# adelacvg/NS2VC

Measured on NVIDIA H100. Metric: denoiser-steps/s, higher is better.
Workload: dtype f32 (3xBF16-split tensor-core contractions, fp32 accumulate)

## Files before the change

ns2vc_b200/csrc/common.cuh:

```cuda
#pragma once
#include <cuda_runtime.h>
#include <cuda_bf16.h>
#include <stdint.h>
#include <stddef.h>

namespace ns2vc {

void set_error(const char* fmt, ...);
const char* get_error();

#define NS_CHECK_CUDA(expr)                                                                    \
  do {                                                                                         \
    cudaError_t _e = (expr);                                                                   \
    if (_e != cudaSuccess) {                                                                   \
      ns2vc::set_error("%s:%d CUDA error %s: %s", __FILE__, __LINE__, cudaGetErrorName(_e),    \
                       cudaGetErrorString(_e));                                                \
      return -2;                                                                               \
    }                                                                                          \
  } while (0)

#define NS_REQUIRE(cond, ...)                                                                  \
  do {                                                                                         \
    if (!(cond)) {                                                                             \
      ns2vc::set_error(__VA_ARGS__);                                                           \
// ... 102 lines not shown
  double* row_stats;
  int f16_col0;
  double* stat_sum;
  double* stat_sq;
  unsigned long long* trace;
  unsigned long long* span;
  int tma_out;
  int bn;
  int xmode;
  int ksplit;
  int nxs;
  XSeg xs[kMaxXSeg];
  const PrepOp* pre;
  const float* pre_film;
  const float* rowmask;
  const int* row_len;
  int len_shift;
  TMap tmap[2 * kMaxSrc];
  TMap tmap_out[3];
};
void plan_gemm(GemmOp& op);
constexpr int kXfMaxC = 1024;
int gemm_sm_count();

int launch_gemm_tc(const GemmOp& op, cudaStream_t st);
int launch_gemm_simt(const GemmOp& op, cudaStream_t st);
int encode_tmaps(GemmOp& op);

struct PackSeg {
  const float* w;
  int n_rows;
  int cin_total;
  int ktaps;
  int tap;
  int cin0, ncin;
  int n_dst0;
  int kb0;
  int nkb;
  int geglu_half;
  const float* cscale;
};
int launch_pack_b(const PackSeg& ps, __nv_bfloat16* w_hi, __nv_bfloat16* w_lo, float* w_f32, int Npad,
                  cudaStream_t st);
int launch_ln_fold_vec(const float* W, const float* gamma, const float* beta, const float* bias, float* g, float* bf, int N, int C, cudaStream_t st);

int launch_prep_split(const PrepOp& op, cudaStream_t st);
// ... 128 lines not shown
```

ns2vc_b200/csrc/gemm_tc.cu:

```cuda
#include "gemm_common.cuh"
#include "prep_common.cuh"
#include "tc_common.cuh"
#include "launch.cuh"
#include <cuda.h>
#include <cuda_fp16.h>
#include <cstdlib>

namespace ns2vc {

constexpr int BM = 128;
constexpr int BK = 64;
constexpr int kEpiWarps = 8;
constexpr int kThreads = (4 + kEpiWarps) * 32;
constexpr int kATileBytes = BM * BK * 2;

constexpr int kMaxStages = 4;
constexpr int kStagePerWarp = 8192;
constexpr int kStageOff = 8192;
constexpr int kStagingBytes = kStageOff + kEpiWarps * kStagePerWarp;

constexpr int kPanelRows = BM + 2;
constexpr int kPanelBytes = 136 * 128;
constexpr int kXAStageBytes = 2 * kPanelBytes;
constexpr int kXBStageBytes = 3 * 2 * (64 * BK * 2);
constexpr int kXAStages = 3;
constexpr int kXBStages = 2;
constexpr int kXOffB = kXAStages * kXAStageBytes;
constexpr int kXOffAff = kXOffB + kXBStages * kXBStageBytes;
constexpr int kXAffBytes = (2 * kXfMaxC + 2 * 64) * 4;

template <int BN_> struct TileCfg {
  static constexpr int BN = BN_;
  static constexpr int kBTileBytes = BN_ * BK * 2;
  static constexpr int kStageBytes = 2 * kATileBytes + 2 * kBTileBytes;
  static constexpr int kStagesSingle = (BN_ == 128) ? 3 : 4;
  static constexpr int kOffAcc = kStagingBytes;
  static constexpr int kPipeBytes = (kStagesSingle * kStageBytes > kXOffAff + kXAffBytes) ? kStagesSingle * kStageBytes : kXOffAff + kXAffBytes;
  static constexpr int kOffBar = kPipeBytes;
  static constexpr int kOffDesc = kOffBar + 1024;
  static constexpr int kOffLnG = kOffDesc + 3072;
  static constexpr int kSmemBytes = kOffLnG + 4096 + 1024 ;
};
static_assert(TileCfg<64>::kSmemBytes <= 227 * 1024 && TileCfg<128>::kSmemBytes <= 227 * 1024, "shared memory budget");
static_assert(kXOffAff + kXAffBytes <= TileCfg<64>::kPipeBytes && kPrepSlots * kEpiWarps * 32 >= kXfMaxC, "panel mode: stages + affine table inside the pipeline area");
constexpr int kXOffAcc = kXOffB + 8 * 256 * 16;
static_assert(kXOffAcc + BM * 64 * 4 <= kXOffAff, "panel mode: parked accumulator inside the weight ring");
static_assert(TileCfg<64>::kOffAcc + BM * 64 * 4 <= TileCfg<64>::kStagesSingle * TileCfg<64>::kStageBytes &&
              TileCfg<128>::kOffAcc + BM * 128 * 4 <= TileCfg<128>::kStagesSingle * TileCfg<128>::kStageBytes, "parked accumulator inside the stage buffers");


__device__ __forceinline__ float* stage_f32_ptr(uint8_t* st, int row, int c4) {
  return reinterpret_cast<float*>(st + row * 128 + ((c4 ^ (row & 7)) << 4));
}


template <bool LNF, bool VOC = false>
__device__ __noinline__ void epi_cold(const GemmOp& op, int b, long long m, int nbase, uint8_t* st, int lane, bool with_gate) {
#pragma unroll 1
  for (int j = 0; j < 32; ++j) {
    float* pv = stage_f32_ptr(st, lane, j >> 2) + (j & 3);
    const float g = with_gate ? reinterpret_cast<const float*>(st + 4096)[lane * 32 + j] : 0.f;
    *pv = (nbase + j < op.n_valid) ? epi_value<LNF, VOC>(op, b, m, nbase + j, *pv, g) : 0.f;
  }
}
__device__ __noinline__ void store_cold(const GemmOp& op, int flags, int b, int t, long long m, int nbase, uint8_t* st, int lane) {
  const bool f16 = nbase >= op.f16_col0;
#pragma unroll 1
  for (int j = 0; j < 32; ++j) {
    const int n = nbase + j;
    if (n >= op.n_valid) break;
    const float v = stage_f32_ptr(st, lane, j >> 2)[j & 3];
// ... 50 lines not shown
      const uint32_t sa = smem_u32(st);
      if (tma & 1) tma_store_3d(&tmo[0], sa, nbase, t_warp0, b);
      if (tma & 2) { tma_store_3d(&tmo[1], sa + 4096u, nbase, t_warp0, b); tma_store_3d(&tmo[2], sa + 6144u, nbase, t_warp0, b); }
      bulk_commit();
    }
  }
  const int direct = ((op.flags & EPI_OUT_NCT) ? EPI_OUT_NCT : 0) | (((op.flags & EPI_OUT_F32) && !(op.tma_out & 1)) ? EPI_OUT_F32 : 0) |
                     (((op.flags & EPI_OUT_SPLIT) && with_split && !(op.tma_out & 2)) ? EPI_OUT_SPLIT : 0);
  if (direct) {
    if (!stage_f32) park_row(st, lane, val);
    if (mv) store_cold(op, direct, b, t, m, nbase, st, lane);
  }
}

__device__ __forceinline__ unsigned long long gtime() { unsigned long long t; asm volatile("mov.u64 %0, %%globaltimer;" : "=l"(t)); return t; }
#define XTRACE(i) do { if (op_param.trace && blockIdx.x == 0 && tid == 128) op_param.trace[16 + (i)] = gtime(); } while (0)
#define TRACE(i) do { if (op.trace && blockIdx.x == 0 && blockIdx.y == 0) op.trace[i] = gtime(); } while (0)
__device__ __forceinline__ long long gclk() { long long t; asm volatile("mov.u64 %0, %%clock64;" : "=l"(t)); return t; }
#define ETRACE(i) do { if (op.trace && blockIdx.x == 0 && blockIdx.y == 0 && warp == 4 && lane == 0) op.trace[8 + (i)] = gclk(); } while (0)

constexpr int kGemmOpHotBytes = (int)offsetof(GemmOp, tmap);
static_assert(kGemmOpHotBytes % 16 == 0 && kGemmOpHotBytes <= 2688 && sizeof(PrepOp) <= 320, "GemmOp's hot part must fit the shared-memory descriptor copy");

template <int BN_, bool LNF, bool XF, bool ENC = false, bool RAG = false, bool VOC = false>
__global__ void __launch_bounds__(kThreads, 1) gemm_tc_kernel(const __grid_constant__ GemmOp op_param) {
  using Cfg = TileCfg<BN_>;
  constexpr int BN = Cfg::BN;
  constexpr int kStageBytes = Cfg::kStageBytes;
  extern __shared__ uint8_t smem_raw[];
  const uint32_t raw = smem_u32(smem_raw);
  const uint32_t base = (raw + 1023u) & ~1023u;
  uint8_t* smem = smem_raw + (base - raw);
  const uint32_t bar_base = base + Cfg::kOffBar;
  auto full_bar = [&](int s) { return bar_base + 8u * s; };
  auto empty_bar = [&](int s) { return bar_base + 8u * (kMaxStages + s); };
  auto b_full = [&](int s) { return bar_base + 8u * (19 + s); };
  auto b_empty = [&](int s) { return bar_base + 8u * (21 + s); };

  const int tid = threadIdx.x, warp = tid >> 5, lane = tid & 31;
  {
    const uint4* src = reinterpret_cast<const uint4*>(&op_param);
    uint4* dst = reinterpret_cast<uint4*>(smem + Cfg::kOffDesc);
    for (int i = tid; i < kGemmOpHotBytes / 16; i += kThreads) dst[i] = src[i];
    if (XF && op_param.xmode && op_param.pre) {
      const uint4* ps = reinterpret_cast<const uint4*>(op_param.pre);
      uint4* pd = reinterpret_cast<uint4*>(smem + Cfg::kOffDesc + 2688);
      for (int i = tid; i < (int)(sizeof(PrepOp) / 16); i += kThreads) pd[i] = __ldg(ps + i);
    }
  }
  const GemmOp& op = *reinterpret_cast<const GemmOp*>(smem + Cfg::kOffDesc);
  const TMap* tmaps = op_param.tmap;
  const int tiles_per_batch = (op_param.T_out + BM - 1) / BM;
  const int n_tiles = op_param.N / BN;
  const int ks = (XF && op_param.xmode && op_param.ksplit > 1) ? op_param.ksplit : 1;
  const int kr = (int)blockIdx.x % ks, bid = (int)blockIdx.x / ks;
  const int nst = Cfg::kStagesSingle;
  uint8_t* stage_area = smem;
  float* acc_tile = reinterpret_cast<float*>(smem + (XF ? kXOffAcc : Cfg::kOffAcc));
  const int wg = (warp - 4) >> 2;
  float acc_d[BN / 2];
#pragma unroll
  for (int i = 0; i < BN / 2; ++i) acc_d[i] = 0.f;
  auto mma3 = [&](uint32_t a_hi, uint32_t a_lo, uint32_t b_hi, uint32_t b_lo) {
    wgmma_bf16<BN>(acc_d, wg_desc(a_hi), wg_desc(b_hi));
    wgmma_bf16<BN>(acc_d, wg_desc(a_lo), wg_desc(b_hi));
    wgmma_bf16<BN>(acc_d, wg_desc(a_hi), wg_desc(b_lo));
  };
  const int nkb = op_param.nkb_total;
  const bool tr0 = blockIdx.x == 0;
  auto xr_ready = [&]() { return bar_base + 8u * 23; };
  auto xr_full = [&]() { return bar_base + 8u * 24; };
  if (tid == 0 && op_param.trace && tr0) op_param.trace[0] = gtime();
  span_begin(op_param.span);

  if (warp == 1 && lane == 0) {
    for (int s = 0; s < kMaxStages; ++s) { mbar_init(full_bar(s), 1); mbar_init(empty_bar(s), kEpiWarps); }
    if (XF) { mbar_init(xr_ready(), 1); mbar_init(xr_full(), kEpiWarps); for (int a = 0; a < kXBStages; ++a) { mbar_init(b_full(a), 1); mbar_init(b_empty(a), kEpiWarps); } }
    mbar_fence_init();
  }
  if (warp == 0 && lane == 0) {
// ... 143 lines not shown
          wgmma_fence();
          for (int j = 0; j < xs.ntap; ++j) {
#pragma unroll
            for (int k = 0; k < BK / 16; ++k) {
              const uint32_t bh = b0 + j * 2 * Cfg::kBTileBytes + k * 32;
              mma3(a_hi + j * 128 + k * 32, a_lo + j * 128 + k * 32, bh, bh + Cfg::kBTileBytes);
            }
          }
          wgmma_commit();
          wgmma_wait<1>();
          if (it > 0 && lane == 0) { mbar_arrive(empty_bar((it - 1) % kXAStages)); mbar_arrive(b_empty((it - 1) % kXBStages)); }
          ++it;
        }
      }
      wgmma_wait<0>();
      XTRACE(4);
    }
  }

  const int npf = nkb < nst ? nkb : nst;
  if constexpr (!xpanel) if (warp == 0 && elect_one()) {
    const int n0 = (bid % n_tiles) * BN;
    for (int kb = 0; kb < npf; ++kb) {
      const uint32_t b_hi = base + kb * kStageBytes + 2 * kATileBytes;
      mbar_arrive_expect_tx(full_bar(kb), 2u * kATileBytes + 2u * Cfg::kBTileBytes);
      const size_t eoff = ((size_t)kb * op.N + n0) * 64;
      bulk_g2s(b_hi, op.w_hi + eoff, Cfg::kBTileBytes, full_bar(kb));
      bulk_g2s(b_hi + Cfg::kBTileBytes, op.w_lo + eoff, Cfg::kBTileBytes, full_bar(kb));
    }
  }
  __syncwarp();

  if (warp == 0) {
    if constexpr (!xpanel) if (elect_one()) {
      const int npre = npf;
      pdl_wait();
      if (tr0) TRACE(2);
      {
        const int mt = bid / n_tiles, n0 = (bid % n_tiles) * BN;
        const int b = mt / tiles_per_batch, t0 = (mt % tiles_per_batch) * BM;
        int si = 0, kbl = 0;
        for (int kb = 0; kb < nkb; ++kb) {
          const int stage = kb % nst;
          const GSeg& s = op.seg[si];
          const uint32_t a_hi = base + stage * kStageBytes;
          const uint32_t a_lo = a_hi + kATileBytes;
          const uint32_t b_hi = a_lo + kATileBytes;
          if (kb >= npre) {
            if (kb >= nst) mbar_wait(empty_bar(stage), (uint32_t)(((kb / nst) & 1) ^ 1));
            mbar_arrive_expect_tx(full_bar(stage), 2u * kATileBytes + 2u * Cfg::kBTileBytes);
            const size_t eoff = ((size_t)kb * op.N + n0) * 64;
            bulk_g2s(b_hi, op.w_hi + eoff, Cfg::kBTileBytes, full_bar(stage));
            bulk_g2s(b_hi + Cfg::kBTileBytes, op.w_lo + eoff, Cfg::kBTileBytes, full_bar(stage));
          }
          const int c = s.c0 + kbl * 64;
          tma_load_3d(a_hi, &tmaps[2 * s.src], c, t0 + s.tap, b, full_bar(stage));
          tma_load_3d(a_lo, &tmaps[2 * s.src + 1], c, t0 + s.tap, b, full_bar(stage));
          if (++kbl == s.nkb) { kbl = 0; ++si; }
        }
      }
    }
  } else if (warp >= 4) {
    pdl_wait();
    __syncwarp();
    const bool leader = elect_one();
    const int q = warp & 3;
    const int r = q * 32 + lane;
    const int cc0 = (warp - 4) >> 2;
    uint8_t* st = stage_area + kStageOff + (warp - 4) * kStagePerWarp;
    const TMap* tmo = op_param.tmap_out;
    bool staged_once = false;
    {
      constexpr int it = 0;
      const int mt = bid / n_tiles, nt = bid % n_tiles, n0 = nt * BN;
      const int b = mt / tiles_per_batch, t0 = (mt % tiles_per_batch) * BM;
      const int t = t0 + r;
      const bool mv = t < op.T_out;
      const long long m = (long long)b * op.T_out + t;
      bool rv = mv;
      if constexpr (RAG) rv = mv && t < ragged_rows(op.row_len, b, op.len_shift);
      if constexpr (VOC) if (op.flags & EPI_ROWMASK) rv = mv && __ldg(op.rowmask + m) != 0.f;
      if constexpr (!xpanel) {
        for (int kb = 0; kb < nkb; ++kb) {
          const int stage = kb % nst;
          mbar_wait(full_bar(stage), (uint32_t)((kb / nst) & 1));
          if (kb == 0 && tr0 && warp == 4 && lane == 0) TRACE(3);
          const uint32_t a_hi = base + stage * kStageBytes + wg * 64 * 128;
          const uint32_t a_lo = a_hi + kATileBytes;
          const uint32_t b_hi = base + stage * kStageBytes + 2 * kATileBytes;
          wgmma_fence();
#pragma unroll
          for (int k = 0; k < BK / 16; ++k) mma3(a_hi + k * 32, a_lo + k * 32, b_hi + k * 32, b_hi + Cfg::kBTileBytes + k * 32);
          wgmma_commit();
          wgmma_wait<1>();
          if (kb > 0 && lane == 0) mbar_arrive(empty_bar((kb - 1) % nst));
        }
        wgmma_wait<0>();
        if (lane == 0) mbar_arrive(empty_bar((nkb - 1) % nst));
        if (it == 0 && tr0 && warp == 4 && lane == 0) TRACE(4);
      }
      asm volatile("bar.sync 1, 256;" ::: "memory");
      acc_park<BN>(acc_tile, acc_d, wg, tid & 127);
#pragma unroll
      for (int i = 0; i < BN / 2; ++i) acc_d[i] = 0.f;
      asm volatile("bar.sync 1, 256;" ::: "memory");
      const int t_warp0 = t0 + q * 32;
      float pre[32];
      float preg[32];
      bool pre_ok = false;
      float ln_mu = 0.f, ln_rstd = 1.f;
      float* sg = reinterpret_cast<float*>(smem + Cfg::kOffLnG) + (warp - 4) * 128;
      if constexpr (LNF) {
        if (mv) ln_row_stats(op, m, ln_mu, ln_rstd);
        __syncwarp();
        if constexpr (BN == 128) {
          const int nb = nt * 64 + cc0 * 32 + lane;
          const bool ok = nb < op.n_valid;
          sg[lane] = ok ? __ldg(op.ln_g + nb) : 0.f;
          sg[32 + lane] = ok ? __ldg(op.ln_g + op.n_valid + nb) : 0.f;
          sg[64 + lane] = ok ? __ldg(op.bias + nb) : 0.f;
          sg[96 + lane] = ok ? __ldg(op.bias + op.n_valid + nb) : 0.f;
          pre_ok = BN == 128 && nt * 64 + cc0 * 32 + 32 <= op.n_valid;
        } else {
          const int nb = n0 + cc0 * 32 + lane;
          const bool ok = nb < op.n_valid;
          sg[lane] = ok ? __ldg(op.ln_g + nb) : 0.f;
          sg[64 + lane] = (ok && (op.flags & EPI_BIAS)) ? __ldg(op.bias + nb) : 0.f;
          pre_ok = mv && n0 + cc0 * 32 + 32 <= op.n_valid && !(op.flags & (EPI_ROWBIAS | EPI_RESIDUAL));
        }
        __syncwarp();
      }
      if constexpr (!LNF) {
      if constexpr (BN == 128) {
        const int nb = nt * 64 + cc0 * 32;
        if (BN == 128 && nb + 32 <= op.n_valid) {
          pre_ok = true;
          const float4* bv = reinterpret_cast<const float4*>(op.bias + nb);
          const float4* bg = reinterpret_cast<const float4*>(op.bias + op.n_valid + nb);
#pragma unroll
          for (int j = 0; j < 8; ++j) {
            const float4 x = __ldg(bv + j), y = __ldg(bg + j);
            pre[4 * j] = x.x; pre[4 * j + 1] = x.y; pre[4 * j + 2] = x.z; pre[4 * j + 3] = x.w;
            preg[4 * j] = y.x; preg[4 * j + 1] = y.y; preg[4 * j + 2] = y.z; preg[4 * j + 3] = y.w;
          }
        }
      } else {
        const int nb = n0 + cc0 * 32;
        if (mv && nb + 32 <= op.n_valid && !(op.flags & EPI_ROWBIAS) && (!(op.flags & EPI_RESIDUAL) || (op.res_ld & 3) == 0)) {
          pre_ok = true;
#pragma unroll
          for (int j = 0; j < 32; ++j) pre[j] = 0.f;
          if (op.flags & EPI_BIAS) {
            const float4* pb = reinterpret_cast<const float4*>(op.bias + nb);
#pragma unroll
            for (int j = 0; j < 8; ++j) { const float4 v = __ldg(pb + j); pre[4 * j] = v.x; pre[4 * j + 1] = v.y; pre[4 * j + 2] = v.z; pre[4 * j + 3] = v.w; }
          }
          if (op.flags & EPI_RESIDUAL) {
            const float4* pr = reinterpret_cast<const float4*>(op.res + m * op.res_ld + nb);
#pragma unroll
            for (int j = 0; j < 8; ++j) { const float4 v = __ldg(pr + j); pre[4 * j] += v.x; pre[4 * j + 1] += v.y; pre[4 * j + 2] += v.z; pre[4 * j + 3] += v.w; }
          }
        }
      }
      }
      float enc_keep = 1.f;
      if constexpr (ENC) if ((op.flags & EPI_ROWMASK) && mv) enc_keep = __ldg(op.rowmask + m);
      if (it == 0 && tr0 && warp == 4 && lane == 0) TRACE(5);
      if (it == 0 && tr0) ETRACE(0);
      auto wait_staging = [&]() {
        if (staged_once && op.tma_out) {
          if (leader) asm volatile("cp.async.bulk.wait_group.read 0;" ::: "memory");
          __syncwarp();
        }
      };
      if constexpr (BN == 128) {
        {
          const int hh = cc0;
          float val[32], gate[32];
          acc_row32<BN>(acc_tile, r, hh * 32, val);
          acc_row32<BN>(acc_tile, r, 64 + hh * 32, gate);
          const int nbase = nt * 64 + hh * 32;
          if (nbase < op.n_valid) {
            if (!rv) {
#pragma unroll
              for (int j = 0; j < 32; ++j) val[j] = 0.f;
            } else if (pre_ok) {
              if constexpr (LNF) {
#pragma unroll
                for (int j = 0; j < 32; j += 2) {
                  const float v0 = fmaf(ln_rstd, val[j] - ln_mu * sg[j], sg[64 + j]), v1 = fmaf(ln_rstd, val[j + 1] - ln_mu * sg[j + 1], sg[65 + j]);
                  const float g0 = fmaf(ln_rstd, gate[j] - ln_mu * sg[32 + j], sg[96 + j]), g1 = fmaf(ln_rstd, gate[j + 1] - ln_mu * sg[33 + j], sg[97 + j]);
                  upk2(fmul2(pk2(v0, v1), gelu_erf2(pk2(g0, g1))), val[j], val[j + 1]);
                }
              } else {
#pragma unroll
                for (int j = 0; j < 32; j += 2)
                  upk2(fmul2(fadd2(pk2(val[j], val[j + 1]), pk2(pre[j], pre[j + 1])), gelu_erf2(fadd2(pk2(gate[j], gate[j + 1]), pk2(preg[j], preg[j + 1])))),
                       val[j], val[j + 1]);
              }
            } else {
              wait_staging();
              park_row(st, lane, val);
#pragma unroll
              for (int j = 0; j < 8; ++j) reinterpret_cast<float4*>(st + 4096)[lane * 8 + j] = make_float4(gate[4 * j], gate[4 * j + 1], gate[4 * j + 2], gate[4 * j + 3]);
              epi_cold<LNF>(op, b, m, nbase, st, lane, true);
              fetch_row(st, lane, val);
            }
            wait_staging();
            emit_chunk(op, tmo, st, lane, leader, false, b, t, t_warp0, m, mv, nbase, val);
            staged_once = true;
          }
        }
      } else {
        float* sm_part = reinterpret_cast<float*>(stage_area) + (it & 1) * (4 * BN * 2);
        const bool stage_f32 = (op.tma_out & 1) || (op.flags & EPI_STATS);
#pragma unroll 1
        for (int cc = cc0; cc < BN / 32; cc += 2) {
          float acc[32];
          acc_row32<BN>(acc_tile, r, cc * 32, acc);
          if (it == 0 && tr0) ETRACE(1);
          if constexpr (XF) if (ks > 1) {
            const int te = tid - 128;
            if (kr != 0) {
              mbar_wait_cluster(xr_ready(), 0);
              const uint32_t rbase = mapa_u32(base + kXOffB, 0);
#pragma unroll
              for (int j = 0; j < 8; ++j) st_remote_f32x4(rbase + (uint32_t)((j * 256 + te) * 16), acc[4 * j], acc[4 * j + 1], acc[4 * j + 2], acc[4 * j + 3]);
              asm volatile("fence.acq_rel.cluster;" ::: "memory");
              __syncwarp();
              if (lane == 0) mbar_arrive_remote(mapa_u32(xr_full(), 0));
              continue;
            }
            if (warp == 4 && lane == 0) mbar_arrive_remote(mapa_u32(xr_ready(), 1));
            mbar_wait_cluster(xr_full(), 0);
            const float4* xr = reinterpret_cast<const float4*>(smem + kXOffB);
#pragma unroll
            for (int j = 0; j < 8; ++j) {
              const float4 v = xr[j * 256 + te];
              acc[4 * j] += v.x; acc[4 * j + 1] += v.y; acc[4 * j + 2] += v.z; acc[4 * j + 3] += v.w;
            }
          }
          const int nbase = n0 + cc * 32;
// ... 66 lines not shown
              for (int rr = 0; rr < 32; ++rr) { const float v = stage_f32_ptr(st, rr, lane >> 2)[lane & 3]; cs += v; cq += v * v; }
              sm_part[(q * BN + cc * 32 + lane) * 2] = cs;
              sm_part[(q * BN + cc * 32 + lane) * 2 + 1] = cq;
              if (it == 0 && tr0) ETRACE(4);
            }
          } else if (op.flags & EPI_STATS) {
            sm_part[(q * BN + cc * 32 + lane) * 2] = 0.f;
            sm_part[(q * BN + cc * 32 + lane) * 2 + 1] = 0.f;
          }
        }
        if ((op.flags & EPI_STATS) && kr == 0) {
          asm volatile("bar.sync 1, 256;" ::: "memory");
          if (it == 0 && tr0) ETRACE(5);
          const int col = tid - 128;
          if (col < BN && n0 + col < op.n_valid) {
            double cs = 0, cq = 0;
#pragma unroll
            for (int w = 0; w < 4; ++w) { cs += (double)sm_part[(w * BN + col) * 2]; cq += (double)sm_part[(w * BN + col) * 2 + 1]; }
            atomicAdd(op.stat_sum + (long long)b * op.n_valid + n0 + col, cs);
            atomicAdd(op.stat_sq + (long long)b * op.n_valid + n0 + col, cq);
          }
        }
      }
    }
    if (op.tma_out && leader) asm volatile("cp.async.bulk.wait_group.read 0;" ::: "memory");
  }

  if (warp == 4 && lane == 0 && tr0) TRACE(6);
  if (tr0) ETRACE(6);
  __syncthreads();
  if (tr0) ETRACE(7);
  if (tid == 0 && tr0) TRACE(7);
  span_end(op.span);
}

typedef CUresult (*EncodeTiledFn)(CUtensorMap*, CUtensorMapDataType, cuuint32_t, void*, const cuuint64_t*, const cuuint64_t*,
                                  const cuuint32_t*, const cuuint32_t*, CUtensorMapInterleave, CUtensorMapSwizzle,
                                  CUtensorMapL2promotion, CUtensorMapFloatOOBfill);
static EncodeTiledFn get_encode_fn() {
  static EncodeTiledFn fn = nullptr;
  if (!fn) {
    void* p = nullptr;
    cudaDriverEntryPointQueryResult q;
    if (cudaGetDriverEntryPoint("cuTensorMapEncodeTiled", &p, cudaEnableDefault, &q) == cudaSuccess && q == cudaDriverEntryPointSuccess)
      fn = reinterpret_cast<EncodeTiledFn>(p);
  }
// ... 45 lines not shown
  }
  for (int i = 0; i < op.nsrc; ++i) {
    int box_rows = BM;
    if (op.xmode)
      for (int k = 0; k < op.nxs; ++k) if (op.xs[k].src == i && op.xs[k].ntap == 3) box_rows = kPanelRows;
    int rc = encode_one(&op.tmap[2 * i], op.src[i].hi, op.src[i], op.B, box_rows);
    if (rc) return rc;
    rc = encode_one(&op.tmap[2 * i + 1], op.src[i].lo, op.src[i], op.B, box_rows);
    if (rc) return rc;
  }
  return 0;
}

static int sm_count() {
  static int n = 0;
  if (!n) {
    int dev = 0;
    cudaGetDevice(&dev);
    if (cudaDeviceGetAttribute(&n, cudaDevAttrMultiProcessorCount, dev) != cudaSuccess || n <= 0) n = 132;
  }
  return n;
}

template <int BN_, bool LNF, bool XF, bool ENC = false, bool RAG = false, bool VOC = false>
static int launch_bn(const GemmOp& op, cudaStream_t st) {
  using Cfg = TileCfg<BN_>;
  static bool attr_set = false;
  if (!attr_set) {
    cudaError_t e = cudaFuncSetAttribute(gemm_tc_kernel<BN_, LNF, XF, ENC, RAG, VOC>, cudaFuncAttributeMaxDynamicSharedMemorySize, Cfg::kSmemBytes);
    if (e != cudaSuccess) { set_error("gemm_tc: cannot set %d B dynamic smem: %s", Cfg::kSmemBytes, cudaGetErrorString(e)); return -2; }
    attr_set = true;
  }
  const int tiles = op.B * ceil_div(op.T_out, BM) * (op.N / BN_);
  int grid = tiles;
  dim3 cluster(1, 1, 1);
  if (XF && op.xmode && op.ksplit > 1) { grid = tiles * op.ksplit; cluster.x = (unsigned)op.ksplit; }
  cudaError_t e = launch_kc(gemm_tc_kernel<BN_, LNF, XF, ENC, RAG, VOC>, dim3(grid), dim3(kThreads), (size_t)Cfg::kSmemBytes, st, cluster, op);
  if (e != cudaSuccess) { set_error("gemm_tc launch failed: %s", cudaGetErrorString(e)); return -2; }
  return 0;
}

int gemm_sm_count() { return sm_count(); }

void plan_gemm(GemmOp& op) {
  op.bn = (op.flags & EPI_GEGLU) ? 128 : 64;
}

int launch_gemm_tc(const GemmOp& op, cudaStream_t st) {
  if (op.N % 128) { set_error("gemm_tc: packed N=%d is not a multiple of 128", op.N); return -1; }
  const bool lnf = (op.flags & EPI_LNFOLD) != 0;
  const bool rag = op.row_len != nullptr;
  if (rag && (lnf || op.bn != 64 || (op.flags & (EPI_GEGLU | EPI_RELU | EPI_ROWMASK)))) {
    set_error("gemm_tc: ragged row masks need a plain 64-wide tile without a folded LayerNorm");
    return -1;
  }
  if (op.flags & EPI_GELU) {
    if (lnf || rag || op.xmode || op.bn != 64 || (op.flags & (EPI_GEGLU | EPI_RELU))) {
      set_error("gemm_tc: the GELU epilogue needs a plain 64-wide tile without a folded LayerNorm or ReLU");
      return -1;
    }
    if ((op.flags & EPI_ROWMASK) && !op.rowmask) { set_error("gemm_tc: EPI_ROWMASK without a mask"); return -1; }
    if (op.nkb_total <= 0) { set_error("gemm_tc: empty K"); return -1; }
    return launch_bn<64, false, false, false, false, true>(op, st);
  }
  if (op.flags & (EPI_RELU | EPI_ROWMASK)) {
    if (lnf || op.xmode || op.bn != 64 || (op.flags & EPI_GEGLU)) { set_error("gemm_tc: ReLU / row-mask epilogues need a plain 64-wide tile"); return -1; }
    if ((op.flags & EPI_ROWMASK) && !op.rowmask) { set_error("gemm_tc: EPI_ROWMASK without a mask"); return -1; }
    if (op.nkb_total <= 0) { set_error("gemm_tc: empty K"); return -1; }
    return launch_bn<64, false, false, true>(op, st);
  }
  if (op.xmode) {
    if (lnf || op.bn != 64 || op.nxs < 1 || op.nxs > kMaxXSeg) { set_error("gemm_tc: panel mode needs a plain 64-wide tile and 1..%d segments", kMaxXSeg); return -1; }
    if (op.pre == nullptr) { set_error("gemm_tc: panel mode without GroupNorm parameters"); return -1; }
    if (op.ksplit != 1 && op.ksplit != 2) { set_error("gemm_tc: ksplit must be 1 or 2"); return -1; }
    return rag ? launch_bn<64, false, true, false, true>(op, st) : launch_bn<64, false, true>(op, st);
  }
  if (op.nkb_total <= 0) { set_error("gemm_tc: empty K"); return -1; }
  if ((op.bn == 128) != ((op.flags & EPI_GEGLU) != 0)) { set_error("gemm_tc: the 128-wide tile is the GEGLU instantiation (plan_gemm)"); return -1; }
  if (op.bn == 128) return lnf ? launch_bn<128, true, false>(op, st) : launch_bn<128, false, false>(op, st);
  if (op.bn != 64) { set_error("gemm_tc: plan_gemm() was not called"); return -1; }
  if (rag) return launch_bn<64, false, false, false, true>(op, st);
  return lnf ? launch_bn<64, true, false>(op, st) : launch_bn<64, false, false>(op, st);
}

}
```

ns2vc_b200/csrc/kernel_check.cu:

```cuda
#include "engine_host.cuh"
#include "../../include/ns2vc_b200.h"

#include <cstdio>
#include <cstring>
#include <string>
#include <vector>

namespace ns2vc {
namespace {

SplitBuf to_split(const ns2vc_check_split& s) {
  SplitBuf b{};
  b.hi = (__nv_bfloat16*)s.hi; b.lo = (__nv_bfloat16*)s.lo; b.T = s.T; b.C = s.C; b.ld = s.ld; b.bpitch = s.bpitch;
  return b;
}

const PackedRecord* packed_record(int kind, const void* handle) {
  const EngineBase* e = nullptr;
  switch (kind) {
    case 0: e = engine_base((const ns2vc_unet*)handle); break;
    case 1: e = engine_base((const ns2vc_pre*)handle); break;
    case 2: e = engine_base((const ns2vc_cv*)handle); break;
    case 3: e = engine_base((const ns2vc_voc*)handle); break;
    default: set_error("check_packed: engine kind %d (0 denoiser, 1 condition encoders, 2 content encoder, 3 vocoder)", kind); return nullptr;
// ... 95 lines not shown
    } else {
      const int Cg = a->gn_C1 + a->gn_C2;
      NS_REQUIRE(a->gn_C1 >= 1 && a->gn_C2 >= 0 && (a->gn_C2 == 0) == (a->gn_stats2 == nullptr) && Cg <= kXfMaxC,
                 "check_gemm: GroupNorm sources %d + %d channels (up to %d)", a->gn_C1, a->gn_C2, kXfMaxC);
      NS_REQUIRE(a->gn_G >= 1 && a->gn_G <= 64 && Cg % a->gn_G == 0 && a->gn_gamma && a->gn_beta,
                 "check_gemm: GroupNorm of %d channels in %d groups", Cg, a->gn_G);
      NS_REQUIRE(!a->gn_film || a->gn_film_ld >= 2 * Cg, "check_gemm: FiLM rows of %d < %d", a->gn_film_ld, 2 * Cg);
      p.C1 = a->gn_C1; p.C2 = a->gn_C2;
      set_group_norm(p, a->B, a->gn_stats1, a->gn_C1, a->gn_stats2, a->gn_C2, a->T_out, a->gn_G, a->gn_eps, a->gn_gamma, a->gn_beta,
                     nullptr, a->gn_film_ld);
      g.pre_film = a->gn_film;
    }
    p.row_len = a->row_len; p.len_shift = a->len_shift;
    NS_CHECK_CUDA(cudaMallocAsync((void**)&pre_dev, sizeof(PrepOp), st));
    NS_CHECK_CUDA(cudaMemcpyAsync(pre_dev, &p, sizeof(PrepOp), cudaMemcpyHostToDevice, st));
    g.pre = pre_dev;
  }
  plan_gemm(g);
  int rc = encode_tmaps(g);
  if (!rc) rc = launch_gemm_tc(g, st);
  if (pre_dev) NS_CHECK_CUDA(cudaFreeAsync(pre_dev, st));
  if (rc) return rc;
  const bool voc = (f & EPI_GELU) != 0, enc = !voc && (f & (EPI_RELU | EPI_ROWMASK));
  report(desc, desc_len, "gemm_tc<%d,LNF=%d,XF=%d,ENC=%d,RAG=%d,VOC=%d>", g.bn, (f & EPI_LNFOLD) ? 1 : 0, g.xmode ? 1 : 0, enc ? 1 : 0,
         g.row_len ? 1 : 0, voc ? 1 : 0);
  return 0;
}

int ns2vc_check_attention(const ns2vc_check_attn_args* a, char* desc, int desc_len, ns2vc_stream stream) {
  NS_REQUIRE(a, "check_attention: null argument");
  NS_REQUIRE(a->B >= 1 && a->H >= 1 && a->dh >= 1, "check_attention: bad sizes B=%d H=%d dh=%d", a->B, a->H, a->dh);
  NS_REQUIRE(a->out || (a->out_hi && a->out_lo), "check_attention: no output");
  AttnOp op; memset(&op, 0, sizeof(op));
  op.B = a->B; op.H = a->H; op.Tq = a->Tq; op.Tk = a->Tk; op.dh = a->dh; op.scale = a->scale;
  op.bias = a->bias;
  op.out = a->out; op.out_ld = a->out_ld;
  op.out_hi = (__nv_bfloat16*)a->out_hi; op.out_lo = (__nv_bfloat16*)a->out_lo; op.out_split_ld = a->out_split_ld;
  cudaStream_t st = (cudaStream_t)stream;
  if (a->v2) {
    NS_REQUIRE(a->qs.hi && a->qs.lo && a->ks.hi && a->ks.lo && a->vs.hi && a->vs.lo, "check_attention: v2 needs split q / k / v");
    op.v2 = 1;
    op.qs = to_split(a->qs); op.ks = to_split(a->ks); op.vs = to_split(a->vs);
    op.q_c0 = a->q_c0; op.k_c0 = a->k_c0; op.v_c0 = a->v_c0;
    op.key_len = a->key_len; op.key_shift = a->key_shift; op.p_split = a->p_split;
    int rc = encode_attn_tmaps(op);
    if (!rc) rc = launch_attention_v2(op, st);
    if (rc) return rc;
    const bool pf16 = attention_v2_p_fp16() && !op.p_split;
// ... 323 lines not shown
```

Measured before the change: 1789.

## Add persistent tile-loop GEMM variant for short-K launches with more tiles than SMs

Adds a LOOP instantiation of the tensor-core GEMM. For plain launches with at most four K blocks and more tiles than SMs, it launches one CTA per SM, and each CTA walks the tiles with a grid stride. The load warp keeps a global k-block counter so the TMA ring runs continuously across tiles. The epilogue parks accumulators in a swizzled per-warp staging layout and prefetches bias/LN vectors before the MMA loop, so the next tile's loads overlap the current epilogue. This costs one pipeline stage (the ring shrinks to make room for the separate staging area) and adds a wait on outstanding bulk stores between tiles.

```diff
diff --git a/ns2vc_b200/csrc/common.cuh b/ns2vc_b200/csrc/common.cuh
--- a/ns2vc_b200/csrc/common.cuh
+++ b/ns2vc_b200/csrc/common.cuh
@@ -148,6 +148,7 @@
 void plan_gemm(GemmOp& op);
 constexpr int kXfMaxC = 1024;
 int gemm_sm_count();
+bool gemm_tc_loops(const GemmOp& op);
 
 int launch_gemm_tc(const GemmOp& op, cudaStream_t st);
 int launch_gemm_simt(const GemmOp& op, cudaStream_t st);
diff --git a/ns2vc_b200/csrc/gemm_tc.cu b/ns2vc_b200/csrc/gemm_tc.cu
--- a/ns2vc_b200/csrc/gemm_tc.cu
+++ b/ns2vc_b200/csrc/gemm_tc.cu
@@ -29,24 +29,60 @@
 constexpr int kXOffAff = kXOffB + kXBStages * kXBStageBytes;
 constexpr int kXAffBytes = (2 * kXfMaxC + 2 * 64) * 4;
 
-template <int BN_> struct TileCfg {
+template <int BN_, bool LOOP = false> struct TileCfg {
   static constexpr int BN = BN_;
   static constexpr int kBTileBytes = BN_ * BK * 2;
   static constexpr int kStageBytes = 2 * kATileBytes + 2 * kBTileBytes;
-  static constexpr int kStagesSingle = (BN_ == 128) ? 3 : 4;
-  static constexpr int kOffAcc = kStagingBytes;
-  static constexpr int kPipeBytes = (kStagesSingle * kStageBytes > kXOffAff + kXAffBytes) ? kStagesSingle * kStageBytes : kXOffAff + kXAffBytes;
+  static constexpr int kStages = LOOP ? ((BN_ == 128) ? 2 : 3) : ((BN_ == 128) ? 3 : 4);
+  static constexpr int kOffRing = LOOP ? kStagingBytes : 0;
+  static constexpr int kOffAcc = LOOP ? kStageOff : kStagingBytes;
+  static constexpr int kRingEnd = kOffRing + kStages * kStageBytes;
+  static constexpr int kPipeBytes = (LOOP || kRingEnd > kXOffAff + kXAffBytes) ? kRingEnd : kXOffAff + kXAffBytes;
   static constexpr int kOffBar = kPipeBytes;
   static constexpr int kOffDesc = kOffBar + 1024;
   static constexpr int kOffLnG = kOffDesc + 3072;
   static constexpr int kSmemBytes = kOffLnG + 4096 + 1024 ;
 };
-static_assert(TileCfg<64>::kSmemBytes <= 227 * 1024 && TileCfg<128>::kSmemBytes <= 227 * 1024, "shared memory budget");
+static_assert(TileCfg<64>::kSmemBytes <= 227 * 1024 && TileCfg<128>::kSmemBytes <= 227 * 1024 &&
+              TileCfg<64, true>::kSmemBytes <= 227 * 1024 && TileCfg<128, true>::kSmemBytes <= 227 * 1024, "shared memory budget");
 static_assert(kXOffAff + kXAffBytes <= TileCfg<64>::kPipeBytes && kPrepSlots * kEpiWarps * 32 >= kXfMaxC, "panel mode: stages + affine table inside the pipeline area");
 constexpr int kXOffAcc = kXOffB + 8 * 256 * 16;
 static_assert(kXOffAcc + BM * 64 * 4 <= kXOffAff, "panel mode: parked accumulator inside the weight ring");
-static_assert(TileCfg<64>::kOffAcc + BM * 64 * 4 <= TileCfg<64>::kStagesSingle * TileCfg<64>::kStageBytes &&
-              TileCfg<128>::kOffAcc + BM * 128 * 4 <= TileCfg<128>::kStagesSingle * TileCfg<128>::kStageBytes, "parked accumulator inside the stage buffers");
+static_assert(TileCfg<64>::kOffAcc + BM * 64 * 4 <= TileCfg<64>::kStages * TileCfg<64>::kStageBytes &&
+              TileCfg<128>::kOffAcc + BM * 128 * 4 <= TileCfg<128>::kStages * TileCfg<128>::kStageBytes, "parked accumulator inside the stage buffers");
+static_assert(BM * 128 * 4 == kEpiWarps * kStagePerWarp && TileCfg<64, true>::kOffRing % 1024 == 0, "tile loop: one staging slot per epilogue warp");
+
+template <int N>
+__device__ __forceinline__ int slot_off(int r, int c) {
+  const int rr = r & 31, slot = ((c & 63) >> 5) * 4 + (r >> 5);
+  const int j = (N == 128 ? ((c >> 6) << 3) : 0) | ((c & 31) >> 2);
+  return slot * (kStagePerWarp / 4) + rr * (N / 2) + ((j ^ (rr & 7)) << 2) + (c & 3);
+}
+template <int N, bool LOOP>
+__device__ __forceinline__ void park_acc(float* tile, const float* d, int g, int t) {
+  if constexpr (!LOOP) {
+    acc_park<N>(tile, d, g, t);
+  } else {
+    const int w = t >> 5, l = t & 31;
+#pragma unroll
+    for (int i = 0; i < N / 2; i += 2) {
+      const int r = 64 * g + 16 * w + (l >> 2) + 8 * ((i >> 1) & 1), c = 8 * (i >> 2) + 2 * (l & 3);
+      *reinterpret_cast<float2*>(tile + slot_off<N>(r, c)) = make_float2(d[i], d[i + 1]);
+    }
+  }
+}
+template <int N, bool LOOP>
+__device__ __forceinline__ void parked_row32(const float* tile, int r, int c0, float* v) {
+  if constexpr (!LOOP) {
+    acc_row32<N>(tile, r, c0, v);
+  } else {
+#pragma unroll
+    for (int j = 0; j < 8; ++j) {
+      const float4 x = *reinterpret_cast<const float4*>(tile + slot_off<N>(r, c0 + 4 * j));
+      v[4 * j] = x.x; v[4 * j + 1] = x.y; v[4 * j + 2] = x.z; v[4 * j + 3] = x.w;
+    }
+  }
+}
 
 
 __device__ __forceinline__ float* stage_f32_ptr(uint8_t* st, int row, int c4) {
@@ -143,9 +179,10 @@
 constexpr int kGemmOpHotBytes = (int)offsetof(GemmOp, tmap);
 static_assert(kGemmOpHotBytes % 16 == 0 && kGemmOpHotBytes <= 2688 && sizeof(PrepOp) <= 320, "GemmOp's hot part must fit the shared-memory descriptor copy");
 
-template <int BN_, bool LNF, bool XF, bool ENC = false, bool RAG = false, bool VOC = false>
+template <int BN_, bool LNF, bool XF, bool ENC = false, bool RAG = false, bool VOC = false, bool LOOP = false>
 __global__ void __launch_bounds__(kThreads, 1) gemm_tc_kernel(const __grid_constant__ GemmOp op_param) {
-  using Cfg = TileCfg<BN_>;
+  static_assert(!(LOOP && XF), "the tile loop is for plain launches");
+  using Cfg = TileCfg<BN_, LOOP>;
   constexpr int BN = Cfg::BN;
   constexpr int kStageBytes = Cfg::kStageBytes;
   extern __shared__ uint8_t smem_raw[];
@@ -173,10 +210,13 @@
   const TMap* tmaps = op_param.tmap;
   const int tiles_per_batch = (op_param.T_out + BM - 1) / BM;
   const int n_tiles = op_param.N / BN;
+  const int n_tiles_all = op_param.B * tiles_per_batch * n_tiles;
+  const int tile_step = LOOP ? (int)gridDim.x : 0;
   const int ks = (XF && op_param.xmode && op_param.ksplit > 1) ? op_param.ksplit : 1;
   const int kr = (int)blockIdx.x % ks, bid = (int)blockIdx.x / ks;
-  const int nst = Cfg::kStagesSingle;
+  const int nst = Cfg::kStages;
   uint8_t* stage_area = smem;
+  const uint32_t ring = base + Cfg::kOffRing;
   float* acc_tile = reinterpret_cast<float*>(smem + (XF ? kXOffAcc : Cfg::kOffAcc));
   const int wg = (warp - 4) >> 2;
   float acc_d[BN / 2];
@@ -366,7 +406,7 @@
   if constexpr (!xpanel) if (warp == 0 && elect_one()) {
     const int n0 = (bid % n_tiles) * BN;
     for (int kb = 0; kb < npf; ++kb) {
-      const uint32_t b_hi = base + kb * kStageBytes + 2 * kATileBytes;
+      const uint32_t b_hi = ring + kb * kStageBytes + 2 * kATileBytes;
       mbar_arrive_expect_tx(full_bar(kb), 2u * kATileBytes + 2u * Cfg::kBTileBytes);
       const size_t eoff = ((size_t)kb * op.N + n0) * 64;
       bulk_g2s(b_hi, op.w_hi + eoff, Cfg::kBTileBytes, full_bar(kb));
@@ -380,18 +420,19 @@
       const int npre = npf;
       pdl_wait();
       if (tr0) TRACE(2);
-      {
-        const int mt = bid / n_tiles, n0 = (bid % n_tiles) * BN;
+      int kg = 0;
+      for (int tile = bid;; tile += tile_step) {
+        const int mt = tile / n_tiles, n0 = (tile % n_tiles) * BN;
         const int b = mt / tiles_per_batch, t0 = (mt % tiles_per_batch) * BM;
         int si = 0, kbl = 0;
         for (int kb = 0; kb < nkb; ++kb) {
-          const int stage = kb % nst;
+          const int g = kg + kb, stage = g % nst;
           const GSeg& s = op.seg[si];
-          const uint32_t a_hi = base + stage * kStageBytes;
+          const uint32_t a_hi = ring + stage * kStageBytes;
           const uint32_t a_lo = a_hi + kATileBytes;
           const uint32_t b_hi = a_lo + kATileBytes;
-          if (kb >= npre) {
-            if (kb >= nst) mbar_wait(empty_bar(stage), (uint32_t)(((kb / nst) & 1) ^ 1));
+          if (g >= npre) {
+            if (g >= nst) mbar_wait(empty_bar(stage), (uint32_t)(((g / nst) & 1) ^ 1));
             mbar_arrive_expect_tx(full_bar(stage), 2u * kATileBytes + 2u * Cfg::kBTileBytes);
             const size_t eoff = ((size_t)kb * op.N + n0) * 64;
             bulk_g2s(b_hi, op.w_hi + eoff, Cfg::kBTileBytes, full_bar(stage));
@@ -402,6 +443,8 @@
           tma_load_3d(a_lo, &tmaps[2 * s.src + 1], c, t0 + s.tap, b, full_bar(stage));
           if (++kbl == s.nkb) { kbl = 0; ++si; }
         }
+        kg += nkb;
+        if (!LOOP || tile + tile_step >= n_tiles_all) break;
       }
     }
   } else if (warp >= 4) {
@@ -413,10 +456,10 @@
     const int cc0 = (warp - 4) >> 2;
     uint8_t* st = stage_area + kStageOff + (warp - 4) * kStagePerWarp;
     const TMap* tmo = op_param.tmap_out;
-    bool staged_once = false;
-    {
-      constexpr int it = 0;
-      const int mt = bid / n_tiles, nt = bid % n_tiles, n0 = nt * BN;
+    for (int it = 0;; ++it) {
+      const int tile = bid + it * tile_step, kg = it * nkb;
+      bool staged_once = false;
+      const int mt = tile / n_tiles, nt = tile % n_tiles, n0 = nt * BN;
       const int b = mt / tiles_per_batch, t0 = (mt % tiles_per_batch) * BM;
       const int t = t0 + r;
       const bool mv = t < op.T_out;
@@ -424,89 +467,109 @@
       bool rv = mv;
       if constexpr (RAG) rv = mv && t < ragged_rows(op.row_len, b, op.len_shift);
       if constexpr (VOC) if (op.flags & EPI_ROWMASK) rv = mv && __ldg(op.rowmask + m) != 0.f;
-      if constexpr (!xpanel) {
-        for (int kb = 0; kb < nkb; ++kb) {
-          const int stage = kb % nst;
-          mbar_wait(full_bar(stage), (uint32_t)((kb / nst) & 1));
-          if (kb == 0 && tr0 && warp == 4 && lane == 0) TRACE(3);
-          const uint32_t a_hi = base + stage * kStageBytes + wg * 64 * 128;
-          const uint32_t a_lo = a_hi + kATileBytes;
-          const uint32_t b_hi = base + stage * kStageBytes + 2 * kATileBytes;
-          wgmma_fence();
-#pragma unroll
-          for (int k = 0; k < BK / 16; ++k) mma3(a_hi + k * 32, a_lo + k * 32, b_hi + k * 32, b_hi + Cfg::kBTileBytes + k * 32);
-          wgmma_commit();
-          wgmma_wait<1>();
-          if (kb > 0 && lane == 0) mbar_arrive(empty_bar((kb - 1) % nst));
-        }
-        wgmma_wait<0>();
-        if (lane == 0) mbar_arrive(empty_bar((nkb - 1) % nst));
-        if (it == 0 && tr0 && warp == 4 && lane == 0) TRACE(4);
-      }
-      asm volatile("bar.sync 1, 256;" ::: "memory");
-      acc_park<BN>(acc_tile, acc_d, wg, tid & 127);
-#pragma unroll
-      for (int i = 0; i < BN / 2; ++i) acc_d[i] = 0.f;
-      asm volatile("bar.sync 1, 256;" ::: "memory");
-      const int t_warp0 = t0 + q * 32;
       float pre[32];
       float preg[32];
       bool pre_ok = false;
       float ln_mu = 0.f, ln_rstd = 1.f;
       float* sg = reinterpret_cast<float*>(smem + Cfg::kOffLnG) + (warp - 4) * 128;
-      if constexpr (LNF) {
-        if (mv) ln_row_stats(op, m, ln_mu, ln_rstd);
-        __syncwarp();
+      auto epi_vectors = [&]() {
+        if constexpr (LNF) {
+          if (mv) ln_row_stats(op, m, ln_mu, ln_rstd);
+          __syncwarp();
+          if constexpr (BN == 128) {
+            const int nb = nt * 64 + cc0 * 32 + lane;
+            const bool ok = nb < op.n_valid;
+            sg[lane] = ok ? __ldg(op.ln_g + nb) : 0.f;
+            sg[32 + lane] = ok ? __ldg(op.ln_g + op.n_valid + nb) : 0.f;
+            sg[64 + lane] = ok ? __ldg(op.bias + nb) : 0.f;
+            sg[96 + lane] = ok ? __ldg(op.bias + op.n_valid + nb) : 0.f;
+            pre_ok = BN == 128 && nt * 64 + cc0 * 32 + 32 <= op.n_valid;
+          } else {
+            const int nb = n0 + cc0 * 32 + lane;
+            const bool ok = nb < op.n_valid;
+            sg[lane] = ok ? __ldg(op.ln_g + nb) : 0.f;
+            sg[64 + lane] = (ok && (op.flags & EPI_BIAS)) ? __ldg(op.bias + nb) : 0.f;
+            pre_ok = mv && n0 + cc0 * 32 + 32 <= op.n_valid && !(op.flags & (EPI_ROWBIAS | EPI_RESIDUAL));
+          }
+          __syncwarp();
+        }
+        if constexpr (!LNF) {
         if constexpr (BN == 128) {
-          const int nb = nt * 64 + cc0 * 32 + lane;
-          const bool ok = nb < op.n_valid;
-          sg[lane] = ok ? __ldg(op.ln_g + nb) : 0.f;
-          sg[32 + lane] = ok ? __ldg(op.ln_g + op.n_valid + nb) : 0.f;
-          sg[64 + lane] = ok ? __ldg(op.bias + nb) : 0.f;
-          sg[96 + lane] = ok ? __ldg(op.bias + op.n_valid + nb) : 0.f;
-          pre_ok = BN == 128 && nt * 64 + cc0 * 32 + 32 <= op.n_valid;
+          const int nb = nt * 64 + cc0 * 32;
+          if (LOOP && nb + 32 <= op.n_valid) {
+            pre_ok = true;
+            sg[64 + lane] = __ldg(op.bias + nb + lane);
+            sg[96 + lane] = __ldg(op.bias + op.n_valid + nb + lane);
+            __syncwarp();
+          } else if (BN == 128 && nb + 32 <= op.n_valid) {
+            pre_ok = true;
+            const float4* bv = reinterpret_cast<const float4*>(op.bias + nb);
+            const float4* bg = reinterpret_cast<const float4*>(op.bias + op.n_valid + nb);
+#pragma unroll
+            for (int j = 0; j < 8; ++j) {
+              const float4 x = __ldg(bv + j), y = __ldg(bg + j);
+              pre[4 * j] = x.x; pre[4 * j + 1] = x.y; pre[4 * j + 2] = x.z; pre[4 * j + 3] = x.w;
+              preg[4 * j] = y.x; preg[4 * j + 1] = y.y; preg[4 * j + 2] = y.z; preg[4 * j + 3] = y.w;
+            }
+          }
         } else {
-          const int nb = n0 + cc0 * 32 + lane;
-          const bool ok = nb < op.n_valid;
-          sg[lane] = ok ? __ldg(op.ln_g + nb) : 0.f;
-          sg[64 + lane] = (ok && (op.flags & EPI_BIAS)) ? __ldg(op.bias + nb) : 0.f;
-          pre_ok = mv && n0 + cc0 * 32 + 32 <= op.n_valid && !(op.flags & (EPI_ROWBIAS | EPI_RESIDUAL));
-        }
+          const int nb = n0 + cc0 * 32;
+          if (mv && nb + 32 <= op.n_valid && !(op.flags & EPI_ROWBIAS) && (!(op.flags & EPI_RESIDUAL) || (op.res_ld & 3) == 0)) {
+            pre_ok = true;
+#pragma unroll
+            for (int j = 0; j < 32; ++j) pre[j] = 0.f;
+            if (op.flags & EPI_BIAS) {
+              const float4* pb = reinterpret_cast<const float4*>(op.bias + nb);
+#pragma unroll
+              for (int j = 0; j < 8; ++j) { const float4 v = __ldg(pb + j); pre[4 * j] = v.x; pre[4 * j + 1] = v.y; pre[4 * j + 2] = v.z; pre[4 * j + 3] = v.w; }
+            }
+            if (op.flags & EPI_RESIDUAL) {
+              const float4* pr = reinterpret_cast<const float4*>(op.res + m * op.res_ld + nb);
+#pragma unroll
+              for (int j = 0; j < 8; ++j) { const float4 v = __ldg(pr + j); pre[4 * j] += v.x; pre[4 * j + 1] += v.y; pre[4 * j + 2] += v.z; pre[4 * j + 3] += v.w; }
+            }
+          }
+        }
+        }
+      };
+      constexpr bool kEarlyVectors = LOOP && (LNF || BN == 128);
+      if constexpr (kEarlyVectors) epi_vectors();
+      if constexpr (!xpanel) {
+        if constexpr (LOOP) {
+#pragma unroll
+          for (int i = 0; i < BN / 2; ++i) acc_d[i] = 0.f;
+        }
+        for (int kb = 0; kb < nkb; ++kb) {
+          const int g = kg + kb, stage = g % nst;
+          mbar_wait(full_bar(stage), (uint32_t)((g / nst) & 1));
+          if (g == 0 && tr0 && warp == 4 && lane == 0) TRACE(3);
+          const uint32_t a_hi = ring + stage * kStageBytes + wg * 64 * 128;
+          const uint32_t a_lo = a_hi + kATileBytes;
+          const uint32_t b_hi = ring + stage * kStageBytes + 2 * kATileBytes;
+          wgmma_fence();
+#pragma unroll
+          for (int k = 0; k < BK / 16; ++k) mma3(a_hi + k * 32, a_lo + k * 32, b_hi + k * 32, b_hi + Cfg::kBTileBytes + k * 32);
+          wgmma_commit();
+          wgmma_wait<1>();
+          if (kb > 0 && lane == 0) mbar_arrive(empty_bar((g - 1) % nst));
+        }
+        wgmma_wait<0>();
+        if (lane == 0) mbar_arrive(empty_bar((kg + nkb - 1) % nst));
+        if (it == 0 && tr0 && warp == 4 && lane == 0) TRACE(4);
+      }
+      if constexpr (LOOP) if (it > 0) {
+        if (op.tma_out && leader) asm volatile("cp.async.bulk.wait_group.read 0;" ::: "memory");
         __syncwarp();
       }
-      if constexpr (!LNF) {
-      if constexpr (BN == 128) {
-        const int nb = nt * 64 + cc0 * 32;
-        if (BN == 128 && nb + 32 <= op.n_valid) {
-          pre_ok = true;
-          const float4* bv = reinterpret_cast<const float4*>(op.bias + nb);
-          const float4* bg = reinterpret_cast<const float4*>(op.bias + op.n_valid + nb);
-#pragma unroll
-          for (int j = 0; j < 8; ++j) {
-            const float4 x = __ldg(bv + j), y = __ldg(bg + j);
-            pre[4 * j] = x.x; pre[4 * j + 1] = x.y; pre[4 * j + 2] = x.z; pre[4 * j + 3] = x.w;
-            preg[4 * j] = y.x; preg[4 * j + 1] = y.y; preg[4 * j + 2] = y.z; preg[4 * j + 3] = y.w;
-          }
-        }
-      } else {
-        const int nb = n0 + cc0 * 32;
-        if (mv && nb + 32 <= op.n_valid && !(op.flags & EPI_ROWBIAS) && (!(op.flags & EPI_RESIDUAL) || (op.res_ld & 3) == 0)) {
-          pre_ok = true;
-#pragma unroll
-          for (int j = 0; j < 32; ++j) pre[j] = 0.f;
-          if (op.flags & EPI_BIAS) {
-            const float4* pb = reinterpret_cast<const float4*>(op.bias + nb);
-#pragma unroll
-            for (int j = 0; j < 8; ++j) { const float4 v = __ldg(pb + j); pre[4 * j] = v.x; pre[4 * j + 1] = v.y; pre[4 * j + 2] = v.z; pre[4 * j + 3] = v.w; }
-          }
-          if (op.flags & EPI_RESIDUAL) {
-            const float4* pr = reinterpret_cast<const float4*>(op.res + m * op.res_ld + nb);
-#pragma unroll
-            for (int j = 0; j < 8; ++j) { const float4 v = __ldg(pr + j); pre[4 * j] += v.x; pre[4 * j + 1] += v.y; pre[4 * j + 2] += v.z; pre[4 * j + 3] += v.w; }
-          }
-        }
+      asm volatile("bar.sync 1, 256;" ::: "memory");
+      park_acc<BN, LOOP>(acc_tile, acc_d, wg, tid & 127);
+      if constexpr (!LOOP) {
+#pragma unroll
+        for (int i = 0; i < BN / 2; ++i) acc_d[i] = 0.f;
       }
-      }
+      asm volatile("bar.sync 1, 256;" ::: "memory");
+      const int t_warp0 = t0 + q * 32;
+      if constexpr (!kEarlyVectors) epi_vectors();
       float enc_keep = 1.f;
       if constexpr (ENC) if ((op.flags & EPI_ROWMASK) && mv) enc_keep = __ldg(op.rowmask + m);
       if (it == 0 && tr0 && warp == 4 && lane == 0) TRACE(5);
@@ -521,8 +584,9 @@
         {
           const int hh = cc0;
           float val[32], gate[32];
-          acc_row32<BN>(acc_tile, r, hh * 32, val);
-          acc_row32<BN>(acc_tile, r, 64 + hh * 32, gate);
+          parked_row32<BN, LOOP>(acc_tile, r, hh * 32, val);
+          parked_row32<BN, LOOP>(acc_tile, r, 64 + hh * 32, gate);
+          if constexpr (LOOP) __syncwarp();
           const int nbase = nt * 64 + hh * 32;
           if (nbase < op.n_valid) {
             if (!rv) {
@@ -536,6 +600,11 @@
                   const float g0 = fmaf(ln_rstd, gate[j] - ln_mu * sg[32 + j], sg[96 + j]), g1 = fmaf(ln_rstd, gate[j + 1] - ln_mu * sg[33 + j], sg[97 + j]);
                   upk2(fmul2(pk2(v0, v1), gelu_erf2(pk2(g0, g1))), val[j], val[j + 1]);
                 }
+              } else if constexpr (LOOP) {
+#pragma unroll
+                for (int j = 0; j < 32; j += 2)
+                  upk2(fmul2(fadd2(pk2(val[j], val[j + 1]), pk2(sg[64 + j], sg[65 + j])), gelu_erf2(fadd2(pk2(gate[j], gate[j + 1]), pk2(sg[96 + j], sg[97 + j])))),
+                       val[j], val[j + 1]);
               } else {
 #pragma unroll
                 for (int j = 0; j < 32; j += 2)
@@ -561,7 +630,7 @@
 #pragma unroll 1
         for (int cc = cc0; cc < BN / 32; cc += 2) {
           float acc[32];
-          acc_row32<BN>(acc_tile, r, cc * 32, acc);
+          parked_row32<BN, LOOP>(acc_tile, r, cc * 32, acc);
           if (it == 0 && tr0) ETRACE(1);
           if constexpr (XF) if (ks > 1) {
             const int te = tid - 128;
@@ -674,6 +743,7 @@
           }
         }
       }
+      if (!LOOP || tile + tile_step >= n_tiles_all) break;
     }
     if (op.tma_out && leader) asm volatile("cp.async.bulk.wait_group.read 0;" ::: "memory");
   }
@@ -765,25 +835,36 @@
   return n;
 }
 
-template <int BN_, bool LNF, bool XF, bool ENC = false, bool RAG = false, bool VOC = false>
+static int gemm_tiles(const GemmOp& op) { return op.B * ceil_div(op.T_out, BM) * (op.N / op.bn); }
+
+template <int BN_, bool LNF, bool XF, bool ENC = false, bool RAG = false, bool VOC = false, bool LOOP = false>
 static int launch_bn(const GemmOp& op, cudaStream_t st) {
-  using Cfg = TileCfg<BN_>;
+  using Cfg = TileCfg<BN_, LOOP>;
   static bool attr_set = false;
   if (!attr_set) {
-    cudaError_t e = cudaFuncSetAttribute(gemm_tc_kernel<BN_, LNF, XF, ENC, RAG, VOC>, cudaFuncAttributeMaxDynamicSharedMemorySize, Cfg::kSmemBytes);
+    cudaError_t e = cudaFuncSetAttribute(gemm_tc_kernel<BN_, LNF, XF, ENC, RAG, VOC, LOOP>, cudaFuncAttributeMaxDynamicSharedMemorySize, Cfg::kSmemBytes);
     if (e != cudaSuccess) { set_error("gemm_tc: cannot set %d B dynamic smem: %s", Cfg::kSmemBytes, cudaGetErrorString(e)); return -2; }
     attr_set = true;
   }
-  const int tiles = op.B * ceil_div(op.T_out, BM) * (op.N / BN_);
-  int grid = tiles;
+  const int tiles = gemm_tiles(op);
+  int grid = (LOOP && tiles > sm_count()) ? sm_count() : tiles;
   dim3 cluster(1, 1, 1);
   if (XF && op.xmode && op.ksplit > 1) { grid = tiles * op.ksplit; cluster.x = (unsigned)op.ksplit; }
-  cudaError_t e = launch_kc(gemm_tc_kernel<BN_, LNF, XF, ENC, RAG, VOC>, dim3(grid), dim3(kThreads), (size_t)Cfg::kSmemBytes, st, cluster, op);
+  cudaError_t e = launch_kc(gemm_tc_kernel<BN_, LNF, XF, ENC, RAG, VOC, LOOP>, dim3(grid), dim3(kThreads), (size_t)Cfg::kSmemBytes, st, cluster, op);
   if (e != cudaSuccess) { set_error("gemm_tc launch failed: %s", cudaGetErrorString(e)); return -2; }
   return 0;
 }
 
 int gemm_sm_count() { return sm_count(); }
+
+constexpr int kLoopMaxKb = 4;
+bool gemm_tc_loops(const GemmOp& op) {
+  return !op.xmode && !(op.flags & (EPI_GELU | EPI_RELU | EPI_ROWMASK)) && op.nkb_total <= kLoopMaxKb && gemm_tiles(op) > sm_count();
+}
+template <int BN_, bool LNF, bool RAG = false>
+static int launch_plain(const GemmOp& op, cudaStream_t st) {
+  return gemm_tc_loops(op) ? launch_bn<BN_, LNF, false, false, RAG, false, true>(op, st) : launch_bn<BN_, LNF, false, false, RAG>(op, st);
+}
 
 void plan_gemm(GemmOp& op) {
   op.bn = (op.flags & EPI_GEGLU) ? 128 : 64;
@@ -820,10 +901,10 @@
   }
   if (op.nkb_total <= 0) { set_error("gemm_tc: empty K"); return -1; }
   if ((op.bn == 128) != ((op.flags & EPI_GEGLU) != 0)) { set_error("gemm_tc: the 128-wide tile is the GEGLU instantiation (plan_gemm)"); return -1; }
-  if (op.bn == 128) return lnf ? launch_bn<128, true, false>(op, st) : launch_bn<128, false, false>(op, st);
+  if (op.bn == 128) return lnf ? launch_plain<128, true>(op, st) : launch_plain<128, false>(op, st);
   if (op.bn != 64) { set_error("gemm_tc: plan_gemm() was not called"); return -1; }
-  if (rag) return launch_bn<64, false, false, false, true>(op, st);
-  return lnf ? launch_bn<64, true, false>(op, st) : launch_bn<64, false, false>(op, st);
-}
-
-}
+  if (rag) return launch_plain<64, false, true>(op, st);
+  return lnf ? launch_plain<64, true>(op, st) : launch_plain<64, false>(op, st);
+}
+
+}
diff --git a/ns2vc_b200/csrc/kernel_check.cu b/ns2vc_b200/csrc/kernel_check.cu
--- a/ns2vc_b200/csrc/kernel_check.cu
+++ b/ns2vc_b200/csrc/kernel_check.cu
@@ -141,8 +141,8 @@
   if (pre_dev) NS_CHECK_CUDA(cudaFreeAsync(pre_dev, st));
   if (rc) return rc;
   const bool voc = (f & EPI_GELU) != 0, enc = !voc && (f & (EPI_RELU | EPI_ROWMASK));
-  report(desc, desc_len, "gemm_tc<%d,LNF=%d,XF=%d,ENC=%d,RAG=%d,VOC=%d>", g.bn, (f & EPI_LNFOLD) ? 1 : 0, g.xmode ? 1 : 0, enc ? 1 : 0,
-         g.row_len ? 1 : 0, voc ? 1 : 0);
+  report(desc, desc_len, "gemm_tc<%d,LNF=%d,XF=%d,ENC=%d,RAG=%d,VOC=%d%s>", g.bn, (f & EPI_LNFOLD) ? 1 : 0, g.xmode ? 1 : 0, enc ? 1 : 0,
+         g.row_len ? 1 : 0, voc ? 1 : 0, gemm_tc_loops(g) ? ",LOOP=1" : "");
   return 0;
 }
 
```

After: 1811, median of 6. 1.3% higher.
